# USTC-StarTeam/DR4SR

Hardware: AMD Instinct MI355X
Metric: training sequences/sec, SASRec d=64 L=50 (higher is better)
Workload: dtype f32; 1 GPU; SASRec on amazon-toys-shaped synthetic rows (BASELINE configs[1]): N=11925, L=50, d=64, 2 layers, 2 heads, FFN 128, dropout 0.50, B=256 rows/GPU/step, toys histogram (10.9% valid) seqlen; global_batch=256, seq_len=50, parallelism=dp1, hip_graph=True, steps_per_graph=30

## Files before the change

dr4sr_amd/csrc/kernels.h:

```cpp
#pragma once
#include <hip/hip_runtime.h>
#include <stdint.h>
#include "../../include/dr4sr_hip.h"
#include "../../include/dr4sr_hip_hooks.h"
#include "prep_body.h"

#define DR4SR_MAX_LAYERS 8

struct LayerWs {
    float* qkv;
    float* ctx;
    float* attn_st;
    unsigned* attn_keep;
    float* u1;
    float* y;
    float* st1;
    float* a;
    float* h;
    float* u2;
    float* st2;
    float* df;
    float* da;
    float* du1;
    float* dout;
    float* dqkv;
};

struct Workspace {
    int64_t off[2 + 12 * DR4SR_MAX_LAYERS];
    int64_t n_params;
    int Tmax;
    int* cu;
    bool scale, attn_split;
    bool attn_tile_sa;
    int* len_buf;
    int* seq_class;
    float* attn_rd;
    int* tile_seq;
    float* X[DR4SR_MAX_LAYERS + 1];
    float* dX[DR4SR_MAX_LAYERS + 1];
// ... 53 lines not shown
    const float* dz; const float* w2T; const float* w1T; const float* out_wT;
    float* df; float* da; float* du1; float* dout; float* dctx;
    float* rd; int n_head;
    float* ln_part;
    const int* state; uint64_t seed; float p; float eps; int layer; int training;
    uint32_t sP, sA, sF;
    unsigned long long* stamps;
    const float* nx_in_w; const float* nx_in_b; float* nx_qkv;
    const float* up_dqkv; const float* up_in_w; const float* up_du1;
    const float* up_kv_part;
    TileAttnArgs at;
    int xcd;
    float* nx_dqkv_zero;
    float* dn_dqkv_zero;
    int wt_attn;
    const unsigned short* sp;
};

struct EmbQkvArgs {
    const float* E; const float* P; const int64_t* idx; const int64_t* rows; const int* cu; const int* tile_seq; float* X;
    const float* W; const float* bias; float* QKV; const int* state;
    int B, L, n_items, training; uint64_t seed; float p;
    int* idx32;
    int2* tok; float* dqkv_zero;
    int xcd;
    int wf_layers;
    const unsigned short* sp;
};
struct QkvEmbBwdArgs {
    const float* dQKV; const float* W; const float* dU1; const int64_t* idx; const int64_t* rows; const int* cu; const int* tile_seq;
// ... 123 lines not shown
```

dr4sr_amd/csrc/linear.hip:

```cpp
#include "common.h"
#include "kernels.h"
#include <cstdlib>
#define STAMP(i) do { if (A.stamps && blockIdx.x == 0 && threadIdx.x == 0) A.stamps[i] = __builtin_amdgcn_s_memtime(); } while (0)

extern __shared__ __attribute__((aligned(16))) float smem[];

__global__ __launch_bounds__(256) void k_transpose(const float* __restrict__ params, float* __restrict__ wT,
                                                   int64_t o_in, int64_t o_out, int64_t o_w1, int64_t o_w2,
                                                   int64_t layer_stride, int64_t wT_stride, int D, int F) {
    const int m = blockIdx.y, layer = blockIdx.z;
    const float* src;
    float* dst = wT + layer * wT_stride;
    int R, C;
    if (m == 0) { src = params + o_in + layer * layer_stride; R = 3 * D; C = D; }
    else if (m == 1) { src = params + o_out + layer * layer_stride; R = D; C = D; dst += 3 * D * D; }
    else if (m == 2) { src = params + o_w1 + layer * layer_stride; R = F; C = D; dst += 4 * D * D; }
    else { src = params + o_w2 + layer * layer_stride; R = D; C = F; dst += 4 * D * D + D * F; }
    for (int i = blockIdx.x * 256 + threadIdx.x; i < R * C; i += gridDim.x * 256) {
        const int r = i / C, c = i % C;
        dst[c * R + r] = src[i];
    }
}

int launch_transpose_weights(const dr4sr_sasrec_plan* p, const Workspace& ws, hipStream_t s) {
// ... 243 lines not shown
    A.sp = wsplit_of(p, ws, 0); A.wf_layers = 0;
    if (wfrag_img_on(p, ws)) { A.sp = reinterpret_cast<const unsigned short*>(ws.wfrag); A.wf_layers = p->n_layer; }
    const bool in_tile = attn_in_tile(p, ws);
    A.tok = (in_tile || ws.attn_tile_sa || attn_wave_on(p, ws)) ? ws.tok : nullptr; A.dqkv_zero = in_tile ? ws.layer[0].dqkv : nullptr;
    A.xcd = tile_xcd_order(p, ws) ? 1 : 0;
    if (A.xcd) grid.x = xcd_grid((int)grid.x, bm);
    if (wave_tiles(p, ws)) return launch_wt_embqkv_fwd(A, ws.Tmax, s);
#define EQ(B_) do { if (D == 64) hipLaunchKernelGGL((k_embqkv_fwd<B_, 64>), grid, blk, lds, s, A); \
                    else hipLaunchKernelGGL((k_embqkv_fwd<B_, 128>), grid, blk, lds, s, A); } while (0)
    BM_DISPATCH(bm, EQ);
#undef EQ
    return DR4SR_LAUNCH_CHECK();
}


template <int BM, int D, bool RES_IN_LDS, bool COPY_LDS>
__device__ __forceinline__ void ln_rowpass(const float* __restrict__ Cs, int ldc, const float* res, int ldres,
                                           const float* __restrict__ lnw, const float* __restrict__ lnb, float eps,
                                           float* __restrict__ U, float* __restrict__ OUT, float* __restrict__ ST,
                                           float* Ls, int ldl, int t0, int T, bool dodrop, const RngKey& rk,
                                           uint32_t site, float4 (*yreg)[D / 64] = nullptr) {
    constexpr int NV = D / 64, PASSES = BM / 16;
    const int l16 = threadIdx.x & 15, rsub = threadIdx.x >> 4;
    float4 gam[NV], bet[NV], v[PASSES][NV];
    float mean[PASSES], rstd[PASSES];
#pragma unroll
    for (int j = 0; j < NV; ++j) { gam[j] = ld4(lnw + 4 * l16 + 64 * j); bet[j] = ld4(lnb + 4 * l16 + 64 * j); }
#pragma unroll
    for (int ps = 0; ps < PASSES; ++ps) {
        const int row = ps * 16 + rsub, t = t0 + row;
        const bool ok = t < T;
#pragma unroll
        for (int j = 0; j < NV; ++j) {
            const int c = 4 * l16 + 64 * j;
            float4 o = ld4(Cs + row * ldc + c);
            float4 r = make_float4(0.f, 0.f, 0.f, 0.f);
            if (RES_IN_LDS) r = ld4(res + row * ldres + c);
            else if (ok) r = ld4(res + (size_t)t * ldres + c);
            if (dodrop) { const float4 m = drop4(rk, site, (uint64_t)t * D + c); o.x *= m.x; o.y *= m.y; o.z *= m.z; o.w *= m.w; }
            v[ps][j] = make_float4(r.x + o.x, r.y + o.y, r.z + o.z, r.w + o.w);
            if (ok) st4(U + (size_t)t * D + c, v[ps][j]);
        }
    }
#pragma unroll
    for (int ps = 0; ps < PASSES; ++ps) ln_stats16<NV>(v[ps], mean[ps], rstd[ps], eps);
#pragma unroll
    for (int ps = 0; ps < PASSES; ++ps) {
        const int row = ps * 16 + rsub, t = t0 + row;
        const bool ok = t < T;
#pragma unroll
        for (int j = 0; j < NV; ++j) {
            const int c = 4 * l16 + 64 * j;
            const float m = mean[ps], rs = rstd[ps];
            const float4 yv = make_float4((v[ps][j].x - m) * rs * gam[j].x + bet[j].x, (v[ps][j].y - m) * rs * gam[j].y + bet[j].y,
                                          (v[ps][j].z - m) * rs * gam[j].z + bet[j].z, (v[ps][j].w - m) * rs * gam[j].w + bet[j].w);
            if (ok && OUT) st4(OUT + (size_t)t * D + c, yv);
            if (yreg) yreg[ps][j] = ok ? yv : make_float4(0.f, 0.f, 0.f, 0.f);
            if (COPY_LDS) st4(Ls + row * ldl + c, ok ? yv : make_float4(0.f, 0.f, 0.f, 0.f));
        }
        if (ok && l16 == 0) { ST[2 * (size_t)t] = mean[ps]; ST[2 * (size_t)t + 1] = rstd[ps]; }
    }
}

template <int BM, int D, int F, bool FFN_ONLY, bool KEEPQ = false>
__device__ __forceinline__ void post_fwd_body(const PostArgs& A, const int t0, const int T, float4 (*zreg)[D / 64] = nullptr,
                                              tattn::Keep* keep_out = nullptr) {
    constexpr int LD = D + 4, LF = F + 4, NVF = F / 64, PASSES = BM / 16;
    float* R0 = smem;
    float* R1 = R0 + BM * LD;
    float* R2 = R1 + BM * LD;
    const int l16 = threadIdx.x & 15, rsub = threadIdx.x >> 4;
    const bool dodrop = A.training && A.p > 0.f;
    const RngKey rk = make_rng(A.seed, (uint32_t)A.state[DR4SR_STATE_RNGSTEP], A.p);
    const uint32_t sP = A.sP, sA = A.sA, sF = A.sF;
    const bool actdrop = dodrop && sA != 0xffffffffu;

    constexpr bool PF = BM == 16 && !FFN_ONLY;
    WFragT<PF ? D : 16, PF ? D : 64> f_out;
    WFragT<PF ? D : 16, PF ? F : 64> f_w1;
    WFragT<PF ? F : 16, PF ? D : 64> f_w2;
    WFragT<PF ? D : 16, PF ? 3 * D : 64> f_nx;
// ... 47 lines not shown
                    tattn::fwd_stage<D, KEEPQ>(A, t0, T, smem + att_lds_off(D, F), att_pre);
                    const tattn::Keep k = tattn::fwd_compute<D, KEEPQ>(A, t0, T, R0, LD, smem + att_lds_off(D, F), att_pre);
                    if (keep_out) *keep_out = k;
                }
            }
        }
        lds_barrier(); STAMP(1);
        {
            TileAcc<BM, D> acc;
            tile_zero(acc);
            if constexpr (PF) tile_mma_frag<BM, D, D>(R0, LD, f_out, acc);
            else tile_gemm<BM == 32 && (D == 128 || FFN_ONLY), BM, D, D>(R0, LD, A.out_w, D, false, A.sp, WSplitGeo<D, F>::E, WSplitGeo<D, F>::OUT, acc);
            tile_to_lds<BM, D>(acc, R2, LD, A.out_b);
        }
        lds_barrier(); STAMP(2);
        ln_rowpass<BM, D, false, true>(R2, LD, A.x, D, A.ln1_w, A.ln1_b, A.eps, A.u1, A.y, A.st1, R1, LD, t0, T, dodrop, rk, sP);
    }
    lds_barrier(); STAMP(3);
    {
        TileAcc<BM, F> acc;
        tile_zero(acc);
        if constexpr (PF) tile_mma_frag<BM, D, F>(R1, LD, f_w1, acc);
        else tile_gemm<BM == 32 && (D == 128 || FFN_ONLY), BM, D, F>(R1, LD, A.w1, D, false, A.sp, WSplitGeo<D, F>::E, WSplitGeo<D, F>::W1, acc);
        tile_to_lds<BM, F>(acc, R2, LF, A.b1);
    }
    lds_barrier(); STAMP(4);
    {
        float4 av[PASSES][NVF];
#pragma unroll
        for (int ps = 0; ps < PASSES; ++ps)
#pragma unroll
            for (int j = 0; j < NVF; ++j) av[ps][j] = ld4(R2 + (ps * 16 + rsub) * LF + 4 * l16 + 64 * j);
#pragma unroll
        for (int ps = 0; ps < PASSES; ++ps) {
            const int row = ps * 16 + rsub, t = t0 + row;
            const bool ok = t < T;
#pragma unroll
            for (int j = 0; j < NVF; ++j) {
                const int c = 4 * l16 + 64 * j;
                const float4 a4 = av[ps][j];
                float4 h = make_float4(gelu_erf(a4.x), gelu_erf(a4.y), gelu_erf(a4.z), gelu_erf(a4.w));
                if (actdrop) { const float4 m = drop4(rk, sA, (uint64_t)t * F + c); h.x *= m.x; h.y *= m.y; h.z *= m.z; h.w *= m.w; }
                if (ok) { st4(A.a + (size_t)t * F + c, a4); st4(A.h + (size_t)t * F + c, h); }
                st4(R2 + row * LF + c, h);
            }
        }
    }
    lds_barrier(); STAMP(5);
    {
        TileAcc<BM, D> acc;
        tile_zero(acc);
        if constexpr (PF) tile_mma_frag<BM, F, D>(R2, LF, f_w2, acc);
        else tile_gemm<BM == 32 && (D == 128 || FFN_ONLY), BM, F, D>(R2, LF, A.w2, F, false, A.sp, WSplitGeo<D, F>::E, WSplitGeo<D, F>::W2, acc);
        tile_to_lds<BM, D>(acc, R0, LD, A.b2);
    }
    lds_barrier(); STAMP(6);
    if (!FFN_ONLY && A.nx_qkv) {
        ln_rowpass<BM, D, true, true>(R0, LD, R1, LD, A.ln2_w, A.ln2_b, A.eps, A.u2, A.z, A.st2, R1, LD, t0, T, dodrop, rk, sF);
        lds_barrier();
        TileAcc<BM, 3 * D> acc;
        tile_zero(acc);
        if constexpr (PF) tile_mma_frag<BM, D, 3 * D>(R1, LD, f_nx, acc);
        else tile_gemm<BM == 32 && (D == 128 || FFN_ONLY), BM, D, 3 * D>(R1, LD, A.nx_in_w, D, false, A.sp ? A.sp + 4 * WSplitGeo<D, F>::E : nullptr, WSplitGeo<D, F>::E, 0, acc);
        tile_to_global<BM, 3 * D>(acc, A.nx_qkv, 3 * D, A.nx_in_b, t0, T);
        if (A.nx_dqkv_zero) zero_kv_rows<BM, D>(A.nx_dqkv_zero, t0, T);
    } else {
        ln_rowpass<BM, D, true, false>(R0, LD, R1, LD, A.ln2_w, A.ln2_b, A.eps, A.u2, A.z, A.st2, nullptr, 0, t0, T, dodrop, rk, sF, zreg);
    }
    STAMP(15);
}

template <int BM, int D, int F, bool FFN_ONLY>
__global__ __launch_bounds__(256) void k_post_fwd(const PostArgs A) {
    const int T = A.state[DR4SR_STATE_T], t0 = xcd_tile(T, BM, A.xcd) * BM;
    if (t0 >= T) return;
    post_fwd_body<BM, D, F, FFN_ONLY>(A, t0, T);
}

template <int NV>
__device__ __forceinline__ void flush_affine(const float4 (&dgam)[NV], const float4 (&dbet)[NV], float* scr, float* dst) {
    constexpr int D = 64 * NV;
    const int l16 = threadIdx.x & 15, lane = threadIdx.x & 63, w = threadIdx.x >> 6;
    auto fold = [&](float v) { v += __shfl_xor(v, 16, 64); v += __shfl_xor(v, 32, 64); return v; };
#pragma unroll
    for (int j = 0; j < NV; ++j) {
        const int c = 4 * l16 + 64 * j;
        const float4 a = make_float4(fold(dgam[j].x), fold(dgam[j].y), fold(dgam[j].z), fold(dgam[j].w));
        const float4 b = make_float4(fold(dbet[j].x), fold(dbet[j].y), fold(dbet[j].z), fold(dbet[j].w));
        if (lane < 16) { st4(scr + w * 2 * D + c, a); st4(scr + w * 2 * D + D + c, b); }
    }
    lds_barrier();
    for (int i = threadIdx.x; i < 2 * D; i += 256)
        dst[i] = (scr[i] + scr[2 * D + i]) + (scr[4 * D + i] + scr[6 * D + i]);
    lds_barrier();
}

template <int BM, int D, int SRC>
__device__ __forceinline__ void ln_bwd_rowpass(const float* __restrict__ Gg, const float* La,
                                               const float* Lb, int ldl, const float* __restrict__ Ug,
                                               const float* __restrict__ ST, const float* __restrict__ lnw,
                                               float* __restrict__ DUg, float* DUl, float* __restrict__ DMg,
                                               float* DMl, float4 (&dgam)[D / 64], float4 (&dbet)[D / 64],
                                               int t0, int T, bool dodrop, const RngKey& rk, uint32_t site,
                                               const float4 (*greg)[D / 64] = nullptr) {
    constexpr int NV = D / 64, PASSES = BM / 16;
    const int l16 = threadIdx.x & 15, rsub = threadIdx.x >> 4;
    float4 gam[NV], g[PASSES][NV], u[PASSES][NV];
    float mean[PASSES], rstd[PASSES];
#pragma unroll
    for (int j = 0; j < NV; ++j) {
        gam[j] = ld4(lnw + 4 * l16 + 64 * j);
        dgam[j] = make_float4(0.f, 0.f, 0.f, 0.f);
        dbet[j] = make_float4(0.f, 0.f, 0.f, 0.f);
    }
#pragma unroll
    for (int ps = 0; ps < PASSES; ++ps) {
        const int row = ps * 16 + rsub, t = t0 + row;
        const bool ok = t < T;
        mean[ps] = ok ? ST[2 * (size_t)t] : 0.f;
        rstd[ps] = ok ? ST[2 * (size_t)t + 1] : 0.f;
#pragma unroll
        for (int j = 0; j < NV; ++j) {
            const int c = 4 * l16 + 64 * j;
            const float4 z4 = make_float4(0.f, 0.f, 0.f, 0.f);
            u[ps][j] = ok ? ld4(Ug + (size_t)t * D + c) : z4;
            if (SRC == 0) g[ps][j] = ok ? ld4(Gg + (size_t)t * D + c) : z4;
            else if (SRC == 3) g[ps][j] = ok ? greg[ps][j] : z4;
            else {
                const float4 p0 = ld4(La + row * ldl + c);
                float4 p1 = z4;
                if (SRC == 1) p1 = ld4(Lb + row * ldl + c);
                else if (ok) p1 = ld4(Gg + (size_t)t * D + c);
                g[ps][j] = ok ? make_float4(p0.x + p1.x, p0.y + p1.y, p0.z + p1.z, p0.w + p1.w) : z4;
            }
        }
    }
#pragma unroll
    for (int ps = 0; ps < PASSES; ++ps) ln_bwd_row<NV>(g[ps], u[ps], mean[ps], rstd[ps], gam, dgam, dbet);
#pragma unroll
    for (int ps = 0; ps < PASSES; ++ps) {
        const int row = ps * 16 + rsub, t = t0 + row;
        const bool ok = t < T;
#pragma unroll
        for (int j = 0; j < NV; ++j) {
            const int c = 4 * l16 + 64 * j;
            const float4 du = g[ps][j];
            if (DUg && ok) st4(DUg + (size_t)t * D + c, du);
            if (DUl) st4(DUl + row * ldl + c, du);
            float4 dm = du;
            if (dodrop) { const float4 m = drop4(rk, site, (uint64_t)t * D + c); dm.x *= m.x; dm.y *= m.y; dm.z *= m.z; dm.w *= m.w; }
            if (ok) st4(DMg + (size_t)t * D + c, dm);
            st4(DMl + row * ldl + c, dm);
        }
    }
}

template <int BM, int D, int F, bool FFN_ONLY, bool DET = false>
__device__ __forceinline__ void post_bwd_body(const PostArgs& A, const int t0, const int T, const int tile,
                                              const float4 (*dzreg)[D / 64] = nullptr, const tattn::Keep* att_staged = nullptr) {
    constexpr int LD = D + 4, LF = F + 4, NV = D / 64, NVF = F / 64, PASSES = BM / 16;
    float* R1 = smem;
    float* R0 = R1 + BM * LD;
    float* R2 = R0 + BM * LD;
    const int l16 = threadIdx.x & 15, rsub = threadIdx.x >> 4;
    const bool dodrop = A.training && A.p > 0.f;
    const RngKey rk = make_rng(A.seed, (uint32_t)A.state[DR4SR_STATE_RNGSTEP], A.p);
    const uint32_t sP = A.sP, sA = A.sA, sF = A.sF;
    const bool actdrop = dodrop && sA != 0xffffffffu;
    float4 dgam[NV], dbet[NV];
#ifdef DR4SR_BWD_NO_PREFETCH
    constexpr bool PFB = false;
#else
    constexpr bool PFB = BM == 16 && !FFN_ONLY && (D == 64 || D == 128);
#endif
    constexpr bool PF64 = PFB && D == 64, PF128 = PFB && D == 128;
    WFragC<PF64 ? 3 * D : 16, PF64 ? D : 64> fr_up;
    WFragC<PFB ? D : 16, PFB ? F : 64> fr_w2;
    WFragC<PFB ? F : 16, PFB ? D : 64> fr_w1;
    WFragC<PFB ? D : 16, PFB ? D : 64> fr_out;
    constexpr bool AT = BM == 16 && !FFN_ONLY && (D == 64 || D == 128);
    bool at_on = false, at_stage = false;
    tattn::Keep keep{0xffffffffu, 0xffffffffu};
    tattn::Stage<AT ? D : 64, true, true> att_st;
    constexpr int UPQ = AT ? (16 * 3 * D / 4) / 256 : 1;
    float4 updq[UPQ];
    bool up_pre = false;
    if constexpr (AT) {
        at_on = A.at.on != 0;
        at_stage = at_on && !att_staged;
        if (att_staged) keep = *att_staged;
        if (at_on && A.dn_dqkv_zero) zero_kv_rows<BM, D>(A.dn_dqkv_zero, t0, T);
        if (at_stage && A.up_dqkv) {
            up_pre = true;
#pragma unroll
            for (int q = 0; q < UPQ; ++q) {
                const int i = threadIdx.x + 256 * q, row = i / (3 * D / 4), c = (i % (3 * D / 4)) * 4;
                updq[q] = make_float4(0.f, 0.f, 0.f, 0.f);
                if (t0 + row < T) updq[q] = ld4(A.up_dqkv + (size_t)(t0 + row) * 3 * D + c);
            }
            if constexpr (PF64) wfrag_load(fr_up, A.up_in_w, D);
            __builtin_amdgcn_sched_barrier(0);
        }
        if (at_stage) {
            const int2 mq = tattn::own_word(A.at, t0, T);
            att_st.issue(A.at, t0, T, (A.at.on & 4) ? tattn::NEAR0 : 0, tattn::WR);
            __builtin_amdgcn_sched_barrier(0);
            keep = tattn::own_keep(A, mq, t0, T);
            __builtin_amdgcn_sched_barrier(0);
        }
    }
    STAMP(16);
    if constexpr (PFB) { if (!A.up_dqkv) wfrag_load(fr_w2, A.w2, F); else if (PF64 && !up_pre) wfrag_load(fr_up, A.up_in_w, D); }
    auto att_commit = [&]() { if constexpr (AT) { if (at_stage) att_st.commit(tattn::Lds<D>(smem + att_lds_off(D, F)), (A.at.on & 4) ? tattn::NEAR0 : 0, tattn::WR); } };

    if (!FFN_ONLY && A.up_dqkv) {
        constexpr int LQ = 3 * D + 4;
        float* Aq = R0;
// ... 4 lines not shown
                st4(Aq + row * LQ + c, updq[q]);
            }
        } else load_tile_bm<BM, 3 * D>(Aq, LQ, A.up_dqkv, 3 * D, t0, T);
        att_commit();
        lds_barrier();
        if constexpr (AT && DET) {
            det_kv_rows<D>(Aq, LQ, const_cast<float*>(A.up_dqkv), A.up_kv_part, A.at.tok, t0, T);
            lds_barrier();
        }
        TileAcc<BM, D> acc;
        tile_zero(acc);
        if constexpr (PF64) { wfrag_load(fr_w2, A.w2, F); tile_mma_frag<BM, 3 * D, D>(Aq, LQ, fr_up, acc); }
        else { tile_gemm<BM == 32 && (D == 128 || FFN_ONLY), BM, 3 * D, D>(Aq, LQ, A.up_in_w, D, true, A.sp ? A.sp + 4 * WSplitGeo<D, F>::E : nullptr, WSplitGeo<D, F>::E, 0, acc); if constexpr (PF128) wfrag_load(fr_w2, A.w2, F); }
        tile_to_lds<BM, D>(acc, R1, LD, nullptr);
        lds_barrier();
        ln_bwd_rowpass<BM, D, 2>(A.up_du1, R1, nullptr, LD, A.u2, A.st2, A.ln2_w, nullptr, R1, A.df, R0, dgam, dbet, t0, T, dodrop, rk, sF);
    } else if (dzreg) {
        att_commit();
        ln_bwd_rowpass<BM, D, 3>(nullptr, nullptr, nullptr, LD, A.u2, A.st2, A.ln2_w, nullptr, R1, A.df, R0, dgam, dbet, t0, T, dodrop, rk, sF, dzreg);
    } else {
        att_commit();
        ln_bwd_rowpass<BM, D, 0>(A.dz, nullptr, nullptr, LD, A.u2, A.st2, A.ln2_w, nullptr, R1, A.df, R0, dgam, dbet, t0, T, dodrop, rk, sF);
    }
    flush_affine<NV>(dgam, dbet, R2, A.ln_part + (size_t)tile * 4 * D);
    {
        TileAcc<BM, F> acc;
        tile_zero(acc);
        if constexpr (PF64) { wfrag_load(fr_w1, A.w1, D); tile_mma_frag<BM, D, F>(R0, LD, fr_w2, acc); }
        else if constexpr (PF128) { tile_mma_frag<BM, D, F>(R0, LD, fr_w2, acc); wfrag_load(fr_w1, A.w1, D); }
        else tile_gemm<BM == 32 && (D == 128 || FFN_ONLY), BM, D, F>(R0, LD, A.w2, F, true, A.sp, WSplitGeo<D, F>::E, WSplitGeo<D, F>::W2, acc);
        tile_to_lds<BM, F>(acc, R2, LF, nullptr);
    }
    lds_barrier();
#pragma unroll
    for (int ps = 0; ps < PASSES; ++ps) {
        const int row = ps * 16 + rsub, t = t0 + row;
#pragma unroll
        for (int j = 0; j < NVF; ++j) {
            const int c = 4 * l16 + 64 * j;
            float4 d = make_float4(0.f, 0.f, 0.f, 0.f);
            if (t < T) {
                d = ld4(R2 + row * LF + c);
                const float4 av = ld4(A.a + (size_t)t * F + c);
                if (actdrop) { const float4 m = drop4(rk, sA, (uint64_t)t * F + c); d.x *= m.x; d.y *= m.y; d.z *= m.z; d.w *= m.w; }
                d.x *= gelu_erf_grad(av.x); d.y *= gelu_erf_grad(av.y); d.z *= gelu_erf_grad(av.z); d.w *= gelu_erf_grad(av.w);
                st4(A.da + (size_t)t * F + c, d);
            }
            st4(R2 + row * LF + c, d);
        }
    }
    lds_barrier();
    {
        TileAcc<BM, D> acc;
        tile_zero(acc);
        if constexpr (PF64) { wfrag_load(fr_out, A.out_w, D); tile_mma_frag<BM, F, D>(R2, LF, fr_w1, acc); }
        else if constexpr (PF128) { tile_mma_frag<BM, F, D>(R2, LF, fr_w1, acc); wfrag_load(fr_out, A.out_w, D); }
        else tile_gemm<BM == 32 && (D == 128 || FFN_ONLY), BM, F, D>(R2, LF, A.w1, D, true, A.sp, WSplitGeo<D, F>::E, WSplitGeo<D, F>::W1, acc);
        tile_to_lds<BM, D>(acc, R0, LD, nullptr);
    }
    lds_barrier();
    if (FFN_ONLY) {
        constexpr int C4f = D / 4;
        for (int i = threadIdx.x; i < BM * C4f; i += 256) {
            const int row = i / C4f, c = (i % C4f) * 4;
            if (t0 + row < T) {
                const float4 p0 = ld4(R0 + row * LD + c), p1 = ld4(R1 + row * LD + c);
                st4(A.du1 + (size_t)(t0 + row) * D + c, make_float4(p0.x + p1.x, p0.y + p1.y, p0.z + p1.z, p0.w + p1.w));
            }
        }
        return;
    }
    ln_bwd_rowpass<BM, D, 1>(nullptr, R0, R1, LD, A.u1, A.st1, A.ln1_w, A.du1, nullptr, A.dout, R1, dgam, dbet, t0, T, dodrop, rk, sP);
    flush_affine<NV>(dgam, dbet, R2, A.ln_part + (size_t)tile * 4 * D + 2 * D);
    {
        TileAcc<BM, D> acc;
        tile_zero(acc);
        if constexpr (PFB) tile_mma_frag<BM, D, D>(R1, LD, fr_out, acc);
        else tile_gemm<BM == 32 && (D == 128 || FFN_ONLY), BM, D, D>(R1, LD, A.out_w, D, true, A.sp, WSplitGeo<D, F>::E, WSplitGeo<D, F>::OUT, acc);
        tile_to_lds<BM, D>(acc, R0, LD, nullptr);
    }
    lds_barrier();
    constexpr int C4 = D / 4;
    for (int i = threadIdx.x; i < BM * C4; i += 256) {
        const int row = i / C4, c = (i % C4) * 4;
        const bool ok = t0 + row < T;
        const float4 v = ld4(R0 + row * LD + c);
        if (ok && !at_on) st4(A.dctx + (size_t)(t0 + row) * D + c, v);
// ... 7 lines not shown
            if constexpr (AT) { if (at_on && (i % C4) % lph == 0) tattn::Lds<D>(smem + att_lds_off(D, F)).rd[row * 2 + (i % C4) / lph] = d; }
        }
    }
    if constexpr (AT) {
        if (at_on) {
            STAMP(17);
            lds_barrier();
            if (at_stage) tattn::far_rows_if_needed<D>(A.at, tattn::Lds<D>(smem + att_lds_off(D, F)), t0, T);
            STAMP(18);
            tattn::bwd<D, DET>(A, t0, T, R0, LD, smem + att_lds_off(D, F), keep);
        }
    }
    STAMP(26);
}

template <int BM, int D, int F, bool FFN_ONLY, bool DET = false>
__global__ __launch_bounds__(256) void k_post_bwd(const PostArgs A) {
    const int T = A.state[DR4SR_STATE_T], bx = xcd_tile(T, BM, A.xcd), t0 = bx * BM;
    if (t0 >= T) return;
    post_bwd_body<BM, D, F, FFN_ONLY, DET>(A, t0, T, bx);
}

template <int LPT>
__device__ __forceinline__ float lane_group_sum(float v) {
#pragma unroll
    for (int o = LPT / 2; o > 0; o >>= 1) v += __shfl_xor(v, o, 64);
    return v;
}

__device__ __forceinline__ float meta_weight_token(const ScoreTileArgs& S, const float4& q, float lt, int b, int pos, int64_t row, int t,
                                                   int sub, uint32_t step, float4& dzw) {
    constexpr int MD = 64;
    const float* W1 = S.phi;
    const float* b1 = S.phi + MD * MD;
    const float* W2 = b1 + MD;
// ... 387 lines not shown
    }
}

template <int BM, int D, int F, bool META, bool DET = false>
__device__ __forceinline__ void post_mid_body(const PostArgs& A, const ScoreTileArgs& S) {
    const int T = A.state[DR4SR_STATE_T], bx = xcd_tile(T, BM, A.xcd), t0 = bx * BM;
    if (t0 >= T) return;
    if constexpr (BM != 16) { if (S.ent) tile_sort_init<BM>(S, smem + post_lds_floats(D, F, BM) + 8); }
    if constexpr (D == 64) {
        ScorePre<BM> P;
        if constexpr (BM == 16) score_prefetch<BM>(A, S, t0, T, P);
        float4 zreg[BM / 16][1], dzreg[BM / 16][1];
        PostArgs Af = A;
        if (!S.rec) Af.z = nullptr;
        tattn::Keep keep{0xffffffffu, 0xffffffffu};
        post_fwd_body<BM, D, F, false, true>(Af, t0, T, zreg, &keep);
        if constexpr (BM != 16) score_prefetch<BM>(A, S, t0, T, P);
        if constexpr (META) lds_barrier();
        score_tile_regs<BM, META>(A, S, t0, T, bx, P, zreg, dzreg, smem + post_lds_floats(D, F, BM), smem);
        if constexpr (BM != 16) { if (S.ent) tile_sort<BM>(S, bx, t0, T, smem + post_lds_floats(D, F, BM) + 8); }
        post_bwd_body<BM, D, F, false, DET>(A, t0, T, bx, dzreg, &keep);
    } else {
        tattn::Keep keep{0xffffffffu, 0xffffffffu};
        post_fwd_body<BM, D, F, false, true>(A, t0, T, nullptr, &keep);
        __syncthreads();
        score_tile<BM, D, META>(A, S, t0, T, bx, smem + post_lds_floats(D, F, BM) + 8);
        if constexpr (BM != 16) { if (S.ent) tile_sort<BM>(S, bx, t0, T, smem + post_lds_floats(D, F, BM) + 8); }
        __syncthreads();
        post_bwd_body<BM, D, F, false, DET>(A, t0, T, bx, nullptr, &keep);
    }
}
template <int BM, int D, int F, bool META, bool DET = false>
__global__ __launch_bounds__(256) void k_post_mid(const PostArgs A, const ScoreTileArgs S) { post_mid_body<BM, D, F, META, DET>(A, S); }
template <int D, int F>
__global__ __launch_bounds__(256) __attribute__((amdgpu_waves_per_eu(4, 4))) void k_post_mid32(const PostArgs A, const ScoreTileArgs S) {
    post_mid_body<32, D, F, false>(A, S);
// ... 24 lines not shown
        A.nx_in_w = P + poff(ws, layer + 1, P_IN_W); A.nx_in_b = P + poff(ws, layer + 1, P_IN_B); A.nx_qkv = ws.layer[layer + 1].qkv;
        A.up_dqkv = ws.layer[layer + 1].dqkv; A.up_in_w = P + poff(ws, layer + 1, P_IN_W); A.up_du1 = ws.layer[layer + 1].du1;
    }
    A.stamps = DR4SR_XENV("DR4SR_STAMPS") ? reinterpret_cast<unsigned long long*>(ws.dctx) : nullptr;
    A.at.on = attn_in_tile(p, ws) ? 1 : 0;
    A.xcd = tile_xcd_order(p, ws) ? 1 : 0;
    const bool near_ok = p->expected_tokens > 0 && p->expected_tokens <= 16 * (int64_t)p->B;
    if (A.at.on && !DR4SR_XENV("DR4SR_ATTN_TILE_FULL") && ((near_ok && p->D == 128) || DR4SR_XENV("DR4SR_ATTN_TILE_NEAR"))) A.at.on |= 4;
    if (A.at.on && DR4SR_ENV("DR4SR_ATTN_TILE_ATOMICS")) A.at.on |= 2;
    A.at.qkv = lw.qkv; A.at.dqkv = lw.dqkv; A.at.ctx = lw.ctx; A.at.stat = lw.attn_st; A.at.tok = ws.tok; A.at.L = p->L; A.at.keep = lw.attn_keep;
    A.wt_attn = attn_fold_fwd(p, ws) ? 1 : 0;
    A.sp = wsplit_of(p, ws, layer);
    if (wfrag_img_on(p, ws)) A.sp = reinterpret_cast<const unsigned short*>(ws.wfrag + (size_t)layer * ws.wT_stride);
    A.at.kv_part = (A.at.on && ws.det_lat && ws.det_kv) ? ws.det_kv + (size_t)layer * ws.det_kv_layer : nullptr;
    A.up_kv_part = (A.at.kv_part && A.up_dqkv) ? ws.det_kv + (size_t)(layer + 1) * ws.det_kv_layer : nullptr;
    A.nx_dqkv_zero = (A.at.on && A.nx_qkv) ? ws.layer[layer + 1].dqkv : nullptr;
    A.dn_dqkv_zero = (A.at.on && layer > 0) ? ws.layer[layer - 1].dqkv : nullptr;
    return A;
}

static size_t post_lds(int D, int F, int bm = 64) { return sizeof(float) * post_lds_floats(D, F, bm); }

template <int BM>
static int post_launch_bm(const dr4sr_sasrec_plan* p, const Workspace& ws, const PostArgs& A, bool bwd, hipStream_t s) {
    dim3 grid((ws.Tmax + BM - 1) / BM), blk(256);
    if (A.xcd) grid.x = xcd_grid((int)grid.x, BM);
    const size_t lds = (BM == 16 && A.at.on) ? sizeof(float) * att_lds_off(p->D, p->F) + att_lds_bytes(p->D) : post_lds(p->D, p->F, BM);
#define PL(D_, F_) do { if (bwd && BM == 16 && A.at.kv_part) { big_lds((k_post_bwd<BM == 16 ? 16 : 64, D_, F_, false, BM == 16>), lds); \
                                                              hipLaunchKernelGGL((k_post_bwd<BM == 16 ? 16 : 64, D_, F_, false, BM == 16>), grid, blk, lds, s, A); } \
                        else if (bwd) { big_lds(k_post_bwd<BM, D_, F_, false>, lds); hipLaunchKernelGGL((k_post_bwd<BM, D_, F_, false>), grid, blk, lds, s, A); } \
                        else { big_lds(k_post_fwd<BM, D_, F_, false>, lds); hipLaunchKernelGGL((k_post_fwd<BM, D_, F_, false>), grid, blk, lds, s, A); } } while (0)
    if (p->D == 64 && p->F == 128) PL(64, 128);
    else if (p->D == 128 && p->F == 128) PL(128, 128);
    else if (p->D == 64 && p->F == 256) PL(64, 256);
    else return DR4SR_E_SHAPE;
#undef PL
    return DR4SR_LAUNCH_CHECK();
}
template <int BM>
static int post_mid_bm(const dr4sr_sasrec_plan* p, const Workspace& ws, const PostArgs& A, const ScoreTileArgs& S, hipStream_t s) {
    dim3 grid((ws.Tmax + BM - 1) / BM), blk(256);
    if (A.xcd) grid.x = xcd_grid((int)grid.x, BM);
// ... 911 lines not shown
```

dr4sr_amd/csrc/step.hip:

```cpp
#include "common.h"
#include "kernels.h"

#include <atomic>
#include <cstdlib>
#include <mutex>
#include <unordered_map>
void big_lds_impl(const void* kernel, size_t bytes) {
    static std::unordered_map<const void*, size_t> granted;
    static std::mutex mu;
    std::lock_guard<std::mutex> lk(mu);
    size_t& g = granted[kernel];
    if (bytes > g) {
        (void)hipFuncSetAttribute(kernel, hipFuncAttributeMaxDynamicSharedMemorySize, (int)bytes);
        g = bytes;
    }
}

extern "C" int dr4sr_abi_version(void) { return DR4SR_ABI_VERSION; }

static StepFork g_fork = {};
const StepFork& step_fork() {
    if (g_fork.state == 0 && DR4SR_XENV("DR4SR_STREAMS")) {
        hipStreamCaptureMode mode = hipStreamCaptureModeRelaxed;
        (void)hipThreadExchangeStreamCaptureMode(&mode);
// ... 152 lines not shown
    }
    ws->wfrag = D == 128 ? take(ws->wT_stride * p->n_layer) : nullptr;
    ws->wsplit_E = D == 128 ? ws->wT_stride : 0;
    ws->wsplit = ws->wsplit_E ? reinterpret_cast<unsigned short*>(take(2 * ws->wsplit_E * p->n_layer)) : nullptr;
    if (!base && ws->wsplit_E) ws->wsplit = reinterpret_cast<unsigned short*>(1);
    ws->score_part = take(2LL * (p->B > (Tmax + 15) / 16 ? p->B : (Tmax + 15) / 16));
    ws->ln_part = take((int64_t)p->n_layer * ((Tmax + 15) / 16) * 4 * D);
    for (int l = 0; l < p->n_layer; ++l) {
        LayerWs& w = ws->layer[l];
        w.qkv = take(Tmax * 3 * D); w.ctx = take(Tmax * D); w.attn_st = take(Tmax * p->H * 2);
        w.attn_keep = reinterpret_cast<unsigned*>(take(Tmax * p->H * 2));
        w.u1 = take(Tmax * D); w.y = take(Tmax * D); w.st1 = take(Tmax * 2);
        w.a = take(Tmax * F); w.h = take(Tmax * F); w.u2 = take(Tmax * D); w.st2 = take(Tmax * 2);
        w.df = take(Tmax * D); w.da = take(Tmax * F); w.du1 = take(Tmax * D); w.dout = take(Tmax * D); w.dqkv = take(Tmax * 3 * D);
    }
    ws->bytes = o;
    return 0;
}

extern "C" int64_t dr4sr_sasrec_workspace_bytes(const dr4sr_sasrec_plan* plan) {
    if (!plan) return DR4SR_E_ARG;
    dr4sr_sasrec_plan q = *plan;
    q.workspace = nullptr;
    if (q.B <= 0 || q.L <= 0 || q.n_layer <= 0 || q.n_layer > DR4SR_MAX_LAYERS) return DR4SR_E_ARG;
    if (check_shape(&q)) return DR4SR_E_SHAPE;
    Workspace ws;
    carve_workspace(&q, &ws);
    return ws.bytes;
}

// ... 392 lines not shown
```

Before: 2.576 million sequences/s.

## Carry LN stats, activations and dropout keep bits across fused post fwd/bwd

Adds a per-thread RowCarry that keeps layernorm inputs, mean/rstd, FFN pre-activations and dropout keep bits in registers when forward and backward are fused in one tile. The separate backward kernel now prefetches these values up front and reads a saved 16-bit per-lane keep mask instead of regenerating dropout masks with the RNG. Forward kernels write that mask to a new per-layer row_keep buffer. The aim is to remove redundant RNG hashing and scattered global reloads in the backward LN/GELU passes. The cost is more registers per thread and an extra small workspace write.

Measured after the change: 2.630 million sequences/s (median of 6 runs). 1.02x the previous value.

```diff
diff --git a/dr4sr_amd/csrc/kernels.h b/dr4sr_amd/csrc/kernels.h
--- a/dr4sr_amd/csrc/kernels.h
+++ b/dr4sr_amd/csrc/kernels.h
@@ -24,6 +24,7 @@
     float* du1;
     float* dout;
     float* dqkv;
+    unsigned short* row_keep;
 };
 
 struct Workspace {
@@ -107,6 +108,7 @@
     float* nx_dqkv_zero;
     float* dn_dqkv_zero;
     int wt_attn;
+    unsigned short* row_keep;
     const unsigned short* sp;
 };
 
diff --git a/dr4sr_amd/csrc/linear.hip b/dr4sr_amd/csrc/linear.hip
--- a/dr4sr_amd/csrc/linear.hip
+++ b/dr4sr_amd/csrc/linear.hip
@@ -281,13 +281,26 @@
 }
 
 
-template <int BM, int D, bool RES_IN_LDS, bool COPY_LDS>
+struct LnCarry { float4 v; float mean, rstd; uint32_t keep; };
+template <int F>
+struct RowCarry { LnCarry ln1, ln2; float4 a[F / 64]; uint32_t akeep; };
+__host__ __device__ constexpr bool carry_vals(int CARRY) { return CARRY != 0; }
+__host__ __device__ constexpr bool carry_bits(int CARRY) { return CARRY == 1 || CARRY == 3; }
+__device__ __forceinline__ uint32_t keep_bits4(const float4& m) {
+    return (m.x != 0.f ? 1u : 0u) | (m.y != 0.f ? 2u : 0u) | (m.z != 0.f ? 4u : 0u) | (m.w != 0.f ? 8u : 0u);
+}
+__device__ __forceinline__ float4 keep_factors4(const RngKey& k, uint32_t bits) {
+    return make_float4((bits & 1u) ? k.scale : 0.f, (bits & 2u) ? k.scale : 0.f, (bits & 4u) ? k.scale : 0.f, (bits & 8u) ? k.scale : 0.f);
+}
+
+template <int BM, int D, bool RES_IN_LDS, bool COPY_LDS, bool CARRY = false>
 __device__ __forceinline__ void ln_rowpass(const float* __restrict__ Cs, int ldc, const float* res, int ldres,
                                            const float* __restrict__ lnw, const float* __restrict__ lnb, float eps,
                                            float* __restrict__ U, float* __restrict__ OUT, float* __restrict__ ST,
                                            float* Ls, int ldl, int t0, int T, bool dodrop, const RngKey& rk,
-                                           uint32_t site, float4 (*yreg)[D / 64] = nullptr) {
+                                           uint32_t site, float4 (*yreg)[D / 64] = nullptr, LnCarry* cy = nullptr) {
     constexpr int NV = D / 64, PASSES = BM / 16;
+    static_assert(!CARRY || (NV == 1 && PASSES == 1), "the carried row state is one float4 per thread");
     const int l16 = threadIdx.x & 15, rsub = threadIdx.x >> 4;
     float4 gam[NV], bet[NV], v[PASSES][NV];
     float mean[PASSES], rstd[PASSES];
@@ -304,13 +317,17 @@
             float4 r = make_float4(0.f, 0.f, 0.f, 0.f);
             if (RES_IN_LDS) r = ld4(res + row * ldres + c);
             else if (ok) r = ld4(res + (size_t)t * ldres + c);
-            if (dodrop) { const float4 m = drop4(rk, site, (uint64_t)t * D + c); o.x *= m.x; o.y *= m.y; o.z *= m.z; o.w *= m.w; }
+            if (dodrop) {
+                const float4 m = drop4(rk, site, (uint64_t)t * D + c); o.x *= m.x; o.y *= m.y; o.z *= m.z; o.w *= m.w;
+                if constexpr (CARRY) cy->keep = keep_bits4(m);
+            }
             v[ps][j] = make_float4(r.x + o.x, r.y + o.y, r.z + o.z, r.w + o.w);
             if (ok) st4(U + (size_t)t * D + c, v[ps][j]);
         }
     }
 #pragma unroll
     for (int ps = 0; ps < PASSES; ++ps) ln_stats16<NV>(v[ps], mean[ps], rstd[ps], eps);
+    if constexpr (CARRY) { cy->v = v[0][0]; cy->mean = mean[0]; cy->rstd = rstd[0]; }
 #pragma unroll
     for (int ps = 0; ps < PASSES; ++ps) {
         const int row = ps * 16 + rsub, t = t0 + row;
@@ -329,9 +346,15 @@
     }
 }
 
-template <int BM, int D, int F, bool FFN_ONLY, bool KEEPQ = false>
+template <int F>
+__device__ __forceinline__ void row_keep_store(const PostArgs& A, const RowCarry<F>& cy, const int t0, const int T) {
+    static_assert(F == 128, "16 bits per thread");
+    const int t = t0 + (threadIdx.x >> 4);
+    if (t < T) A.row_keep[16 * (size_t)t + (threadIdx.x & 15)] = (unsigned short)(cy.ln1.keep | (cy.ln2.keep << 4) | (cy.akeep << 8));
+}
+template <int BM, int D, int F, bool FFN_ONLY, bool KEEPQ = false, int CARRY = 0>
 __device__ __forceinline__ void post_fwd_body(const PostArgs& A, const int t0, const int T, float4 (*zreg)[D / 64] = nullptr,
-                                              tattn::Keep* keep_out = nullptr) {
+                                              tattn::Keep* keep_out = nullptr, RowCarry<F>* cy = nullptr) {
     constexpr int LD = D + 4, LF = F + 4, NVF = F / 64, PASSES = BM / 16;
     float* R0 = smem;
     float* R1 = R0 + BM * LD;
@@ -409,7 +432,8 @@
             tile_to_lds<BM, D>(acc, R2, LD, A.out_b);
         }
         lds_barrier(); STAMP(2);
-        ln_rowpass<BM, D, false, true>(R2, LD, A.x, D, A.ln1_w, A.ln1_b, A.eps, A.u1, A.y, A.st1, R1, LD, t0, T, dodrop, rk, sP);
+        ln_rowpass<BM, D, false, true, CARRY != 0>(R2, LD, A.x, D, A.ln1_w, A.ln1_b, A.eps, A.u1, A.y, A.st1, R1, LD, t0, T, dodrop, rk, sP, nullptr,
+                                              CARRY ? &cy->ln1 : nullptr);
     }
     lds_barrier(); STAMP(3);
     {
@@ -435,7 +459,11 @@
                 const int c = 4 * l16 + 64 * j;
                 const float4 a4 = av[ps][j];
                 float4 h = make_float4(gelu_erf(a4.x), gelu_erf(a4.y), gelu_erf(a4.z), gelu_erf(a4.w));
-                if (actdrop) { const float4 m = drop4(rk, sA, (uint64_t)t * F + c); h.x *= m.x; h.y *= m.y; h.z *= m.z; h.w *= m.w; }
+                if constexpr (CARRY != 0) { cy->a[j] = a4; if (j == 0) cy->akeep = 0; }
+                if (actdrop) {
+                    const float4 m = drop4(rk, sA, (uint64_t)t * F + c); h.x *= m.x; h.y *= m.y; h.z *= m.z; h.w *= m.w;
+                    if constexpr (CARRY != 0) cy->akeep |= keep_bits4(m) << (4 * j);
+                }
                 if (ok) { st4(A.a + (size_t)t * F + c, a4); st4(A.h + (size_t)t * F + c, h); }
                 st4(R2 + row * LF + c, h);
             }
@@ -451,7 +479,9 @@
     }
     lds_barrier(); STAMP(6);
     if (!FFN_ONLY && A.nx_qkv) {
-        ln_rowpass<BM, D, true, true>(R0, LD, R1, LD, A.ln2_w, A.ln2_b, A.eps, A.u2, A.z, A.st2, R1, LD, t0, T, dodrop, rk, sF);
+        ln_rowpass<BM, D, true, true, CARRY != 0>(R0, LD, R1, LD, A.ln2_w, A.ln2_b, A.eps, A.u2, A.z, A.st2, R1, LD, t0, T, dodrop, rk, sF, nullptr,
+                                                  CARRY ? &cy->ln2 : nullptr);
+        if constexpr (CARRY == 2) row_keep_store<F>(A, *cy, t0, T);
         lds_barrier();
         TileAcc<BM, 3 * D> acc;
         tile_zero(acc);
@@ -460,16 +490,22 @@
         tile_to_global<BM, 3 * D>(acc, A.nx_qkv, 3 * D, A.nx_in_b, t0, T);
         if (A.nx_dqkv_zero) zero_kv_rows<BM, D>(A.nx_dqkv_zero, t0, T);
     } else {
-        ln_rowpass<BM, D, true, false>(R0, LD, R1, LD, A.ln2_w, A.ln2_b, A.eps, A.u2, A.z, A.st2, nullptr, 0, t0, T, dodrop, rk, sF, zreg);
+        ln_rowpass<BM, D, true, false, CARRY != 0>(R0, LD, R1, LD, A.ln2_w, A.ln2_b, A.eps, A.u2, A.z, A.st2, nullptr, 0, t0, T, dodrop, rk, sF, zreg,
+                                                   CARRY ? &cy->ln2 : nullptr);
+        if constexpr (CARRY == 2) row_keep_store<F>(A, *cy, t0, T);
     }
     STAMP(15);
 }
 
-template <int BM, int D, int F, bool FFN_ONLY>
+template <int BM, int D, int F, bool FFN_ONLY, bool KB = false>
 __global__ __launch_bounds__(256) void k_post_fwd(const PostArgs A) {
     const int T = A.state[DR4SR_STATE_T], t0 = xcd_tile(T, BM, A.xcd) * BM;
     if (t0 >= T) return;
-    post_fwd_body<BM, D, F, FFN_ONLY>(A, t0, T);
+    if constexpr (KB) {
+        RowCarry<F> cy;
+        cy.ln1.keep = cy.ln2.keep = cy.akeep = 0;
+        post_fwd_body<BM, D, F, FFN_ONLY, false, 2>(A, t0, T, nullptr, nullptr, &cy);
+    } else post_fwd_body<BM, D, F, FFN_ONLY>(A, t0, T);
 }
 
 template <int NV>
@@ -490,15 +526,17 @@
     lds_barrier();
 }
 
-template <int BM, int D, int SRC>
+template <int BM, int D, int SRC, int CARRY = 0>
 __device__ __forceinline__ void ln_bwd_rowpass(const float* __restrict__ Gg, const float* La,
                                                const float* Lb, int ldl, const float* __restrict__ Ug,
                                                const float* __restrict__ ST, const float* __restrict__ lnw,
                                                float* __restrict__ DUg, float* DUl, float* __restrict__ DMg,
                                                float* DMl, float4 (&dgam)[D / 64], float4 (&dbet)[D / 64],
                                                int t0, int T, bool dodrop, const RngKey& rk, uint32_t site,
-                                               const float4 (*greg)[D / 64] = nullptr) {
+                                               const float4 (*greg)[D / 64] = nullptr, const LnCarry* cy = nullptr) {
     constexpr int NV = D / 64, PASSES = BM / 16;
+    static_assert(!CARRY || (NV == 1 && PASSES == 1), "the carried row state is one float4 per thread");
+    constexpr bool VALS = carry_vals(CARRY), BITS = carry_bits(CARRY);
     const int l16 = threadIdx.x & 15, rsub = threadIdx.x >> 4;
     float4 gam[NV], g[PASSES][NV], u[PASSES][NV];
     float mean[PASSES], rstd[PASSES];
@@ -512,13 +550,14 @@
     for (int ps = 0; ps < PASSES; ++ps) {
         const int row = ps * 16 + rsub, t = t0 + row;
         const bool ok = t < T;
-        mean[ps] = ok ? ST[2 * (size_t)t] : 0.f;
-        rstd[ps] = ok ? ST[2 * (size_t)t + 1] : 0.f;
+        if constexpr (VALS) { mean[ps] = ok ? cy->mean : 0.f; rstd[ps] = ok ? cy->rstd : 0.f; }
+        else { mean[ps] = ok ? ST[2 * (size_t)t] : 0.f; rstd[ps] = ok ? ST[2 * (size_t)t + 1] : 0.f; }
 #pragma unroll
         for (int j = 0; j < NV; ++j) {
             const int c = 4 * l16 + 64 * j;
             const float4 z4 = make_float4(0.f, 0.f, 0.f, 0.f);
-            u[ps][j] = ok ? ld4(Ug + (size_t)t * D + c) : z4;
+            if constexpr (VALS) u[ps][j] = ok ? cy->v : z4;
+            else u[ps][j] = ok ? ld4(Ug + (size_t)t * D + c) : z4;
             if (SRC == 0) g[ps][j] = ok ? ld4(Gg + (size_t)t * D + c) : z4;
             else if (SRC == 3) g[ps][j] = ok ? greg[ps][j] : z4;
             else {
@@ -543,16 +582,21 @@
             if (DUg && ok) st4(DUg + (size_t)t * D + c, du);
             if (DUl) st4(DUl + row * ldl + c, du);
             float4 dm = du;
-            if (dodrop) { const float4 m = drop4(rk, site, (uint64_t)t * D + c); dm.x *= m.x; dm.y *= m.y; dm.z *= m.z; dm.w *= m.w; }
+            if (dodrop) {
+                float4 m;
+                if constexpr (BITS) m = keep_factors4(rk, cy->keep); else m = drop4(rk, site, (uint64_t)t * D + c);
+                dm.x *= m.x; dm.y *= m.y; dm.z *= m.z; dm.w *= m.w;
+            }
             if (ok) st4(DMg + (size_t)t * D + c, dm);
             st4(DMl + row * ldl + c, dm);
         }
     }
 }
 
-template <int BM, int D, int F, bool FFN_ONLY, bool DET = false>
+template <int BM, int D, int F, bool FFN_ONLY, bool DET = false, int CARRY = 0>
 __device__ __forceinline__ void post_bwd_body(const PostArgs& A, const int t0, const int T, const int tile,
-                                              const float4 (*dzreg)[D / 64] = nullptr, const tattn::Keep* att_staged = nullptr) {
+                                              const float4 (*dzreg)[D / 64] = nullptr, const tattn::Keep* att_staged = nullptr,
+                                              const RowCarry<F>* cy_in = nullptr) {
     constexpr int LD = D + 4, LF = F + 4, NV = D / 64, NVF = F / 64, PASSES = BM / 16;
     float* R1 = smem;
     float* R0 = R1 + BM * LD;
@@ -580,6 +624,8 @@
     constexpr int UPQ = AT ? (16 * 3 * D / 4) / 256 : 1;
     float4 updq[UPQ];
     bool up_pre = false;
+    RowCarry<F> cy_ld;
+    const RowCarry<F>* cy = CARRY >= 2 ? &cy_ld : cy_in;
     if constexpr (AT) {
         at_on = A.at.on != 0;
         at_stage = at_on && !att_staged;
@@ -596,6 +642,26 @@
             if constexpr (PF64) wfrag_load(fr_up, A.up_in_w, D);
             __builtin_amdgcn_sched_barrier(0);
         }
+        if constexpr (CARRY >= 2) {
+            static_assert(D == 64 && BM == 16, "one row, one float4 per thread");
+            const int t = t0 + rsub, c = 4 * l16;
+            const bool ok = t < T;
+            const float4 z4 = make_float4(0.f, 0.f, 0.f, 0.f);
+            const float2 z2 = make_float2(0.f, 0.f);
+            cy_ld.ln2.v = ok ? ld4(A.u2 + (size_t)t * D + c) : z4;
+            const float2 s2 = ok ? *reinterpret_cast<const float2*>(A.st2 + 2 * (size_t)t) : z2;
+#pragma unroll
+            for (int j = 0; j < NVF; ++j) cy_ld.a[j] = ok ? ld4(A.a + (size_t)t * F + c + 64 * j) : z4;
+            cy_ld.ln1.v = ok ? ld4(A.u1 + (size_t)t * D + c) : z4;
+            const float2 s1 = ok ? *reinterpret_cast<const float2*>(A.st1 + 2 * (size_t)t) : z2;
+            cy_ld.ln2.mean = s2.x; cy_ld.ln2.rstd = s2.y; cy_ld.ln1.mean = s1.x; cy_ld.ln1.rstd = s1.y;
+            cy_ld.ln1.keep = cy_ld.ln2.keep = cy_ld.akeep = 0;
+            if constexpr (CARRY == 3) {
+                const uint32_t w = ok ? (uint32_t)A.row_keep[16 * (size_t)t + l16] : 0u;
+                cy_ld.ln1.keep = w & 15u; cy_ld.ln2.keep = (w >> 4) & 15u; cy_ld.akeep = w >> 8;
+            }
+            __builtin_amdgcn_sched_barrier(0);
+        }
         if (at_stage) {
             const int2 mq = tattn::own_word(A.at, t0, T);
             att_st.issue(A.at, t0, T, (A.at.on & 4) ? tattn::NEAR0 : 0, tattn::WR);
@@ -630,13 +696,16 @@
         else { tile_gemm<BM == 32 && (D == 128 || FFN_ONLY), BM, 3 * D, D>(Aq, LQ, A.up_in_w, D, true, A.sp ? A.sp + 4 * WSplitGeo<D, F>::E : nullptr, WSplitGeo<D, F>::E, 0, acc); if constexpr (PF128) wfrag_load(fr_w2, A.w2, F); }
         tile_to_lds<BM, D>(acc, R1, LD, nullptr);
         lds_barrier();
-        ln_bwd_rowpass<BM, D, 2>(A.up_du1, R1, nullptr, LD, A.u2, A.st2, A.ln2_w, nullptr, R1, A.df, R0, dgam, dbet, t0, T, dodrop, rk, sF);
+        ln_bwd_rowpass<BM, D, 2, CARRY>(A.up_du1, R1, nullptr, LD, A.u2, A.st2, A.ln2_w, nullptr, R1, A.df, R0, dgam, dbet, t0, T, dodrop, rk, sF, nullptr,
+                                        CARRY ? &cy->ln2 : nullptr);
     } else if (dzreg) {
         att_commit();
-        ln_bwd_rowpass<BM, D, 3>(nullptr, nullptr, nullptr, LD, A.u2, A.st2, A.ln2_w, nullptr, R1, A.df, R0, dgam, dbet, t0, T, dodrop, rk, sF, dzreg);
+        ln_bwd_rowpass<BM, D, 3, CARRY>(nullptr, nullptr, nullptr, LD, A.u2, A.st2, A.ln2_w, nullptr, R1, A.df, R0, dgam, dbet, t0, T, dodrop, rk, sF, dzreg,
+                                        CARRY ? &cy->ln2 : nullptr);
     } else {
         att_commit();
-        ln_bwd_rowpass<BM, D, 0>(A.dz, nullptr, nullptr, LD, A.u2, A.st2, A.ln2_w, nullptr, R1, A.df, R0, dgam, dbet, t0, T, dodrop, rk, sF);
+        ln_bwd_rowpass<BM, D, 0, CARRY>(A.dz, nullptr, nullptr, LD, A.u2, A.st2, A.ln2_w, nullptr, R1, A.df, R0, dgam, dbet, t0, T, dodrop, rk, sF, nullptr,
+                                        CARRY ? &cy->ln2 : nullptr);
     }
     flush_affine<NV>(dgam, dbet, R2, A.ln_part + (size_t)tile * 4 * D);
     {
@@ -657,8 +726,13 @@
             float4 d = make_float4(0.f, 0.f, 0.f, 0.f);
             if (t < T) {
                 d = ld4(R2 + row * LF + c);
-                const float4 av = ld4(A.a + (size_t)t * F + c);
-                if (actdrop) { const float4 m = drop4(rk, sA, (uint64_t)t * F + c); d.x *= m.x; d.y *= m.y; d.z *= m.z; d.w *= m.w; }
+                float4 av;
+                if constexpr (carry_vals(CARRY)) av = cy->a[j]; else av = ld4(A.a + (size_t)t * F + c);
+                if (actdrop) {
+                    float4 m;
+                    if constexpr (carry_bits(CARRY)) m = keep_factors4(rk, cy->akeep >> (4 * j)); else m = drop4(rk, sA, (uint64_t)t * F + c);
+                    d.x *= m.x; d.y *= m.y; d.z *= m.z; d.w *= m.w;
+                }
                 d.x *= gelu_erf_grad(av.x); d.y *= gelu_erf_grad(av.y); d.z *= gelu_erf_grad(av.z); d.w *= gelu_erf_grad(av.w);
                 st4(A.da + (size_t)t * F + c, d);
             }
@@ -686,7 +760,8 @@
         }
         return;
     }
-    ln_bwd_rowpass<BM, D, 1>(nullptr, R0, R1, LD, A.u1, A.st1, A.ln1_w, A.du1, nullptr, A.dout, R1, dgam, dbet, t0, T, dodrop, rk, sP);
+    ln_bwd_rowpass<BM, D, 1, CARRY>(nullptr, R0, R1, LD, A.u1, A.st1, A.ln1_w, A.du1, nullptr, A.dout, R1, dgam, dbet, t0, T, dodrop, rk, sP, nullptr,
+                                    CARRY ? &cy->ln1 : nullptr);
     flush_affine<NV>(dgam, dbet, R2, A.ln_part + (size_t)tile * 4 * D + 2 * D);
     {
         TileAcc<BM, D> acc;
@@ -724,11 +799,12 @@
     STAMP(26);
 }
 
-template <int BM, int D, int F, bool FFN_ONLY, bool DET = false>
+template <int BM, int D, int F, bool FFN_ONLY, bool DET = false, bool KB = false>
 __global__ __launch_bounds__(256) void k_post_bwd(const PostArgs A) {
     const int T = A.state[DR4SR_STATE_T], bx = xcd_tile(T, BM, A.xcd), t0 = bx * BM;
     if (t0 >= T) return;
-    post_bwd_body<BM, D, F, FFN_ONLY, DET>(A, t0, T, bx);
+    constexpr int CARRY = (BM == 16 && D == 64 && !FFN_ONLY) ? (KB ? 3 : 2) : 0;
+    post_bwd_body<BM, D, F, FFN_ONLY, DET, CARRY>(A, t0, T, bx);
 }
 
 template <int LPT>
@@ -1146,12 +1222,14 @@
         PostArgs Af = A;
         if (!S.rec) Af.z = nullptr;
         tattn::Keep keep{0xffffffffu, 0xffffffffu};
-        post_fwd_body<BM, D, F, false, true>(Af, t0, T, zreg, &keep);
+        constexpr int CARRY = BM == 16 ? 1 : 0;
+        RowCarry<F> cy;
+        post_fwd_body<BM, D, F, false, true, CARRY>(Af, t0, T, zreg, &keep, &cy);
         if constexpr (BM != 16) score_prefetch<BM>(A, S, t0, T, P);
         if constexpr (META) lds_barrier();
         score_tile_regs<BM, META>(A, S, t0, T, bx, P, zreg, dzreg, smem + post_lds_floats(D, F, BM), smem);
         if constexpr (BM != 16) { if (S.ent) tile_sort<BM>(S, bx, t0, T, smem + post_lds_floats(D, F, BM) + 8); }
-        post_bwd_body<BM, D, F, false, DET>(A, t0, T, bx, dzreg, &keep);
+        post_bwd_body<BM, D, F, false, DET, CARRY>(A, t0, T, bx, dzreg, &keep, &cy);
     } else {
         tattn::Keep keep{0xffffffffu, 0xffffffffu};
         post_fwd_body<BM, D, F, false, true>(A, t0, T, nullptr, &keep);
@@ -1206,18 +1284,32 @@
     if (wfrag_img_on(p, ws)) A.sp = reinterpret_cast<const unsigned short*>(ws.wfrag + (size_t)layer * ws.wT_stride);
     A.at.kv_part = (A.at.on && ws.det_lat && ws.det_kv) ? ws.det_kv + (size_t)layer * ws.det_kv_layer : nullptr;
     A.up_kv_part = (A.at.kv_part && A.up_dqkv) ? ws.det_kv + (size_t)(layer + 1) * ws.det_kv_layer : nullptr;
+    A.row_keep = lw.row_keep;
     A.nx_dqkv_zero = (A.at.on && A.nx_qkv) ? ws.layer[layer + 1].dqkv : nullptr;
     A.dn_dqkv_zero = (A.at.on && layer > 0) ? ws.layer[layer - 1].dqkv : nullptr;
     return A;
 }
 
 static size_t post_lds(int D, int F, int bm = 64) { return sizeof(float) * post_lds_floats(D, F, bm); }
+
+static bool row_keep_saved(const dr4sr_sasrec_plan* p, const Workspace& ws, const PostArgs& A) {
+    return A.training && p->p_drop > 0.f && p->D == 64 && p->F == 128 && tile_rows(ws) == 16 && !wave_tiles(p, ws) && !DR4SR_ENV("DR4SR_NO_FUSE")
+           && A.row_keep != nullptr;
+}
 
 template <int BM>
 static int post_launch_bm(const dr4sr_sasrec_plan* p, const Workspace& ws, const PostArgs& A, bool bwd, hipStream_t s) {
     dim3 grid((ws.Tmax + BM - 1) / BM), blk(256);
     if (A.xcd) grid.x = xcd_grid((int)grid.x, BM);
     const size_t lds = (BM == 16 && A.at.on) ? sizeof(float) * att_lds_off(p->D, p->F) + att_lds_bytes(p->D) : post_lds(p->D, p->F, BM);
+    if constexpr (BM == 16) {
+        if (row_keep_saved(p, ws, A)) {
+            if (bwd && A.at.kv_part) { big_lds((k_post_bwd<16, 64, 128, false, true, true>), lds); hipLaunchKernelGGL((k_post_bwd<16, 64, 128, false, true, true>), grid, blk, lds, s, A); }
+            else if (bwd) { big_lds((k_post_bwd<16, 64, 128, false, false, true>), lds); hipLaunchKernelGGL((k_post_bwd<16, 64, 128, false, false, true>), grid, blk, lds, s, A); }
+            else { big_lds((k_post_fwd<16, 64, 128, false, true>), lds); hipLaunchKernelGGL((k_post_fwd<16, 64, 128, false, true>), grid, blk, lds, s, A); }
+            return DR4SR_LAUNCH_CHECK();
+        }
+    }
 #define PL(D_, F_) do { if (bwd && BM == 16 && A.at.kv_part) { big_lds((k_post_bwd<BM == 16 ? 16 : 64, D_, F_, false, BM == 16>), lds); \
                                                               hipLaunchKernelGGL((k_post_bwd<BM == 16 ? 16 : 64, D_, F_, false, BM == 16>), grid, blk, lds, s, A); } \
                         else if (bwd) { big_lds(k_post_bwd<BM, D_, F_, false>, lds); hipLaunchKernelGGL((k_post_bwd<BM, D_, F_, false>), grid, blk, lds, s, A); } \
diff --git a/dr4sr_amd/csrc/step.hip b/dr4sr_amd/csrc/step.hip
--- a/dr4sr_amd/csrc/step.hip
+++ b/dr4sr_amd/csrc/step.hip
@@ -190,6 +190,7 @@
         w.a = take(Tmax * F); w.h = take(Tmax * F); w.u2 = take(Tmax * D); w.st2 = take(Tmax * 2);
         w.df = take(Tmax * D); w.da = take(Tmax * F); w.du1 = take(Tmax * D); w.dout = take(Tmax * D); w.dqkv = take(Tmax * 3 * D);
     }
+    for (int l = 0; l < p->n_layer; ++l) ws->layer[l].row_keep = reinterpret_cast<unsigned short*>(take(Tmax * 8));
     ws->bytes = o;
     return 0;
 }
```
